# facebookresearch/brainmagick

Measured on AMD Instinct MI355X. Metric: segments/s, 208-ch x 360-sample SimpleConv + ClipLoss training step, higher is better.
Workload: dtype f32 (fp32-accurate: operands split into 2 scaled f16 planes, 3 MFMA products, fp32 accumulate; same parity tolerances as exact fp32, see DESIGN.md §2); 1 GPU; cfg2: gwilliams2022-shaped MEG C=208 T=360, F=120 features, 27 subjects, clip_conv SimpleConv (8985590 params) + ClipLoss + Adam; batch_per_gpu=256, global_batch=256, negatives=local, parallelism=dp1, comm=none, rccl_world=1, candidate_gather=none, distinct_batches=8

## Files before the change

brainmagick_amd/csrc/clip.hip:

```cpp
#include "bm_common.h"

__global__ __launch_bounds__(256) void inv_norms_kernel(const float* __restrict__ cand, long K,
                                                        float* __restrict__ inv_norm) {
    __shared__ double sh[4];
    const float* row = cand + (long)blockIdx.x * K;
    double s = 0;
    if ((K & 3) == 0) {
        float a0 = 0.f, a1 = 0.f, a2 = 0.f, a3 = 0.f;
        for (long i = threadIdx.x; i < K / 4; i += blockDim.x) {
            const float4 v = reinterpret_cast<const float4*>(row)[i];
            a0 += v.x * v.x; a1 += v.y * v.y; a2 += v.z * v.z; a3 += v.w * v.w;
        }
        s = (double)a0 + (double)a1 + (double)a2 + (double)a3;
    } else {
        float a = 0.f;
        for (long i = threadIdx.x; i < K; i += blockDim.x) a += row[i] * row[i];
        s = a;
    }
    s = bm_wave_sum_d(s);
    if ((threadIdx.x & 63) == 0) sh[threadIdx.x >> 6] = s;
    __syncthreads();
    if (threadIdx.x == 0) {
        const double t = sh[0] + sh[1] + sh[2] + sh[3];
        inv_norm[blockIdx.x] = 1.0f / (1e-8f + (float)sqrt(t));
// ... 359 lines not shown
}

extern "C" int bm_row_softmax(const float* x, float* y, int rows, int cols, void* stream) {
    BM_REQUIRE(x && y, "row_softmax: null pointer");
    if (rows == 0) return BM_OK;
    hipLaunchKernelGGL(row_softmax_kernel, dim3((rows + 3) / 4), dim3(256), 0, (hipStream_t)stream, x, y, rows, cols);
    return bm_check_launch("row_softmax");
}

__global__ __launch_bounds__(256) void rowwise_dot_kernel(const float* __restrict__ a, const float* __restrict__ b,
                                                          const float* __restrict__ scale, float* __restrict__ out,
                                                          long K) {
    __shared__ double sh[4];
    const float* ar = a + (long)blockIdx.x * K;
    const float* br = b + (long)blockIdx.x * K;
    float s = 0.f;
    for (long i = threadIdx.x; i < K; i += blockDim.x) s += ar[i] * br[i];
    double d = bm_wave_sum_d((double)s);
    if ((threadIdx.x & 63) == 0) sh[threadIdx.x >> 6] = d;
    __syncthreads();
    if (threadIdx.x == 0) out[blockIdx.x] = (float)(sh[0] + sh[1] + sh[2] + sh[3]) * (scale ? scale[blockIdx.x] : 1.f);
}

extern "C" int bm_rowwise_dot(const float* a, const float* b, const float* scale, float* out, int rows, long K,
                              void* stream) {
    BM_REQUIRE(a && b && out, "rowwise_dot: null pointer");
    if (rows == 0) return BM_OK;
    hipLaunchKernelGGL(rowwise_dot_kernel, dim3(rows), dim3(256), 0, (hipStream_t)stream, a, b, scale, out, K);
    return bm_check_launch("rowwise_dot");
}

__global__ void segment_sum_cols_kernel(const float* __restrict__ p, const int* __restrict__ order,
                                        const int* __restrict__ seg, float* __restrict__ pv, int rows,
                                        int cols, int V) {
    const int lane = threadIdx.x & 63;
    const int row = blockIdx.x * (blockDim.x >> 6) + (threadIdx.x >> 6);
    if (row >= rows) return;
    const float* pr = p + (long)row * cols;
    for (int v = lane; v < V; v += 64) {
        float s = 0.f;
        for (int k = seg[v]; k < seg[v + 1]; ++k) s += pr[order[k]];
        pv[(long)row * V + v] = s;
    }
}

extern "C" int bm_segment_sum_cols(const float* p, const int* order, const int* seg, float* pv, int rows,
                                   int cols, int V, void* stream) {
    BM_REQUIRE(p && order && seg && pv, "segment_sum_cols: null pointer");
    if (rows == 0 || V == 0) return BM_OK;
    hipLaunchKernelGGL(segment_sum_cols_kernel, dim3((rows + 3) / 4), dim3(256), 0, (hipStream_t)stream, p, order,
                       seg, pv, rows, cols, V);
    return bm_check_launch("segment_sum_cols");
}
```

brainmagick_amd/csrc/pack.hip:

```cpp
#include "bm_common.h"

__global__ void pack_weights_kernel(const float* __restrict__ src, float* __restrict__ dst, int G,
                                    int M, int Cin, int KS, long sg, long sm, long sc, long sj,
                                    int flip, int Mpad, int nchunk, const float* alpha_ptr) {
    const long total = (long)G * nchunk * KS * BM_BKC * Mpad;
    const float alpha = alpha_ptr ? *alpha_ptr : 1.f;
    for (long i = (long)blockIdx.x * blockDim.x + threadIdx.x; i < total;
         i += (long)gridDim.x * blockDim.x) {
        long r = i;
        const int m = (int)(r % Mpad); r /= Mpad;
        const int cc = (int)(r % BM_BKC); r /= BM_BKC;
        const int j = (int)(r % KS); r /= KS;
        const int chunk = (int)(r % nchunk);
        const int g = (int)(r / nchunk);
        const int c = chunk * BM_BKC + cc;
        float v = 0.f;
        if (m < M && c < Cin) {
            const int jj = flip ? KS - 1 - j : j;
            v = alpha * src[g * sg + m * sm + c * sc + jj * sj];
        }
        dst[i] = v;
    }
}

// ... 60 lines not shown

extern "C" int bm_group_by_index(const long* idx, int B, int G, int* order, int* seg, int* err_flag,
                                 void* stream) {
    BM_REQUIRE(seg && ((idx && order) || B == 0), "group_by_index: null pointer");
    BM_REQUIRE(B >= 0 && G > 0, "group_by_index: bad dims B=%d G=%d", B, G);
    BM_REQUIRE((long)G + 1 + B <= BM_GROUP_MAX_INTS, "group_by_index: B + G + 1 = %ld ints of LDS exceed the %d of a "
               "launch (B=%d G=%d)", (long)G + 1 + B, BM_GROUP_MAX_INTS, B, G);
    hipLaunchKernelGGL(group_by_index_kernel, dim3(1), dim3(256), (size_t)(G + 1 + B) * sizeof(int),
                       (hipStream_t)stream, idx, B, G, order, seg, err_flag);
    return bm_check_launch("group_by_index");
}

__global__ void index_to_i32_kernel(const long* __restrict__ idx, int B, int G, int* __restrict__ out,
                                    int* __restrict__ err) {
    const int i = blockIdx.x * blockDim.x + threadIdx.x;
    if (i >= B) return;
    long v = idx[i];
    if (v < 0 || v >= G) {
        if (err) atomicExch(err, 1);
        v = 0;
    }
    out[i] = (int)v;
}

extern "C" int bm_index_to_i32(const long* idx, int B, int G, int* out, int* err_flag, void* stream) {
    BM_REQUIRE((idx && out) || B == 0, "index_to_i32: null pointer");
    BM_REQUIRE(B >= 0 && G > 0, "index_to_i32: bad dims B=%d G=%d", B, G);
    if (B == 0) return BM_OK;
    hipLaunchKernelGGL(index_to_i32_kernel, dim3((B + 255) / 256), dim3(256), 0, (hipStream_t)stream, idx, B,
                       G, out, err_flag);
    return bm_check_launch("index_to_i32");
}

__global__ void reduce_splits_kernel(const float* __restrict__ part, float* __restrict__ out, int G,
                                     int nsplit, int M, int Cn, int KS, long sg, long sm, long sc,
                                     long sj) {
    const long N = (long)Cn * KS;
    const long per = (long)M * N;
    const long total = (long)G * per;
    for (long i = (long)blockIdx.x * blockDim.x + threadIdx.x; i < total;
         i += (long)gridDim.x * blockDim.x) {
        const int g = (int)(i / per);
        const long r = i - (long)g * per;
        const int m = (int)(r / N);
        const int n = (int)(r - (long)m * N);
        const int c = n / KS, j = n - c * KS;
        const float* p = part + (long)g * nsplit * per + r;
        float s = 0.f;
        for (int k = 0; k < nsplit; ++k) s += p[(long)k * per];
        out[g * sg + m * sm + c * sc + j * sj] = s;
    }
}

__global__ void reduce_splits_vec4_kernel(const float* __restrict__ part, float* __restrict__ out, int G,
                                          int nsplit, int M, int Cn, int KS, long sg, long sm, long sc,
                                          long sj) {
    const long N = (long)Cn * KS;
    const long per = (long)M * N;
    const long total4 = (long)G * per / 4;
    for (long i4 = (long)blockIdx.x * blockDim.x + threadIdx.x; i4 < total4;
         i4 += (long)gridDim.x * blockDim.x) {
        const long i = i4 * 4;
        const int g = (int)(i / per);
        const long r = i - (long)g * per;
        const float* p = part + (long)g * nsplit * per + r;
        float4 s = make_float4(0.f, 0.f, 0.f, 0.f);
// ... 62 lines not shown
```

brainmagick_amd/functional.py:

```python

import torch

from . import hip_ops as H



ACT_CODES = {"none": H.ACT_NONE, "gelu": H.ACT_GELU, "relu": H.ACT_RELU, "leaky": H.ACT_LEAKY}


def _c(t: torch.Tensor) -> torch.Tensor:
    return t if t.is_contiguous() else t.contiguous()


_arange_cache = {}


def _arange_i32(n: int, device, repeat: int = 1) -> torch.Tensor:
    key = (n, repeat, device.type, device.index)
    t = _arange_cache.get(key)
    if t is None:
        if len(_arange_cache) > 64:
            _arange_cache.clear()
        t = torch.arange(n, dtype=torch.int32, device=device)
        if repeat != 1:
# ... 219 lines not shown
        U, C, O, D = ctx.dims
        dout = _c(dout)
        B, _, T = meg.shape
        dheads = None
        if ctx.needs_input_grad[1]:
            order, seg = H.group_by_index(_c(layout_index.to(torch.int64)), U)
            dweights = H.gemm_nt(dout, meg, B, O, C, T, 1, 1, order=order, seg=seg, G=U).view(U, O, C)
            dscores = H.softmax_bwd(weights, dweights)
            wp = H.pack_weights(dscores, U, O, C, 1, O * C, C, 1, 0, shape=(D, 1))
            uidx = _arange_i32(U, meg.device)
            _, per_layout, _ = H.conv_nn(emb, wp, O, 1, 1, widx=uidx)
            if ctx.per_layout_heads:
                dheads = per_layout
            else:
                dheads = H.sum_over_batch(per_layout) if U > 1 else per_layout[0]
        dmeg = None
        if ctx.needs_input_grad[0]:
            wpt = H.pack_weights(weights, U, C, O, 1, O * C, 1, C, 0, shape=(T, 1))
            _, dmeg, _ = H.conv_nn(dout, wpt, C, 1, 1, widx=widx)
        return dmeg, dheads, None, None, None, None


class FusedFrontEndFn(torch.autograd.Function):

    @staticmethod
    def forward(ctx, meg, heads, w1, b1, ws, positions_u, layout_index, subjects, ban_center, ban_radius: float):
        meg, heads, w1, ws, positions_u = _c(meg), _c(heads), _c(w1), _c(ws), _c(positions_u)
        U, C, _ = positions_u.shape
        O, Dp = heads.shape
        L = w1.shape[0]
        S, _, D = ws.shape
        B, _, T = meg.shape
        dev = meg.device
        emb = H.fourier_emb(positions_u, Dp)
        seg_u = _arange_i32(U + 1, dev)
        scores = H.gemm_nt(heads, emb, U, O, C, Dp, a_strides=(0, Dp), x_strides=(C * Dp, Dp), seg=seg_u,
                           G=U).view(U, O, C)
        wm = H.masked_softmax(scores, positions_u, ban_center, ban_radius)
        _, p, _ = H.conv_nn(wm, H.pack_conv_fwd(w1), L, 1, 1)
        bcol = (b1 if b1 is not None else torch.zeros(L, device=dev)).view(1, L, 1).expand(U, L, 1)
        xp = torch.cat([p, bcol], dim=2).repeat_interleave(S, dim=0).contiguous()
        widx_p = _arange_i32(S, dev, repeat=U)
        _, wc, _ = H.conv_nn(xp, H.pack_weights(ws, S, D, L, 1, L * D, 1, D, 0), D, 1, 1, widx=widx_p)
        bias_c = wc[:, :, C].contiguous()
        pair = H.index_i32(_c(layout_index.to(torch.int64)), U) * S + H.index_i32(_c(subjects.to(torch.int64)), S)
        wpc = H.pack_weights(wc, U * S, D, C, 1, D * (C + 1), C + 1, 1, 0, shape=(T, 1))
        _, out, _ = H.conv_nn(meg, wpc, D, 1, 1, widx=pair, bias=bias_c, bias_gstride=D)
        ctx.save_for_backward(meg, emb, wm, xp, ws, w1, pair, widx_p, wc)
        ctx.dims = (U, C, O, Dp, L, S, D)
        ctx.has_b1 = b1 is not None
        return out

    @staticmethod
    def backward(ctx, dout):
        meg, emb, wm, xp, ws, w1, pair, widx_p, wc = ctx.saved_tensors
        U, C, O, Dp, L, S, D = ctx.dims
        dout = _c(dout)
        B, _, T = meg.shape
        dev = meg.device
        P = U * S
        order, seg = H.group_by_index(pair.to(torch.int64), P)
        gaug = torch.empty(P, D, C + 1, device=dev, dtype=torch.float32)
        H.gemm_nt(dout, meg, B, D, C, T, 1, 1, order=order, seg=seg, G=P, out=gaug,
                  out_strides=(D * (C + 1), C + 1, 1, 0))
        gaug[:, :, C] = H.segment_sum_cols(H.time_sums_t(dout), order, seg).t()
        seg_p = _arange_i32(P + 1, dev)
        dws = dw1 = db1 = dheads = None
        if ctx.needs_input_grad[4]:
            t1 = H.gemm_nt(xp, gaug, P, L, D, C + 1, seg=seg_p, G=P)
            dws = (H.sum_over_batch(t1.view(U, S * L * D)) if U > 1 else t1).view(S, L, D)
        _, a, _ = H.conv_nn(gaug, H.pack_weights(ws, S, L, D, 1, L * D, D, 1, 0), L, 1, 1, widx=widx_p)
        a_u = torch.stack([H.sum_over_batch(a[u * S:(u + 1) * S]) for u in range(U)])
        if ctx.has_b1 and ctx.needs_input_grad[3]:
            db1 = H.sum_over_batch(a_u[:, :, C].contiguous()) if U > 1 else a_u[0, :, C].contiguous()
        if ctx.needs_input_grad[2]:
            dw1 = H.gemm_nt(a_u, wm, U, L, O, C, 1, 1, a_strides=(L * (C + 1), C + 1),
                            x_strides=(O * C, C)).view(L, O, 1)
        if ctx.needs_input_grad[1]:
            _, dwm, _ = H.conv_nn(a_u, H.pack_conv_dgrad(w1), O, 1, 1)
            dscores = H.softmax_bwd(wm, dwm[:, :, :C].contiguous())
            wp = H.pack_weights(dscores, U, O, C, 1, O * C, C, 1, 0, shape=(Dp, 1))
            uidx = _arange_i32(U, dev)
            _, per_layout, _ = H.conv_nn(emb, wp, O, 1, 1, widx=uidx)
            dheads = H.sum_over_batch(per_layout) if U > 1 else per_layout[0]
        dmeg = None
        if ctx.needs_input_grad[0]:
            wpt = H.pack_weights(wc, P, C, D, 1, D * (C + 1), 1, C + 1, 0, shape=(T, 1))
            _, dmeg, _ = H.conv_nn(dout, wpt, C, 1, 1, widx=pair)
        return dmeg, dheads, dw1, db1, dws, None, None, None, None, None


_CLIP_BLOCK_BYTES = 0x3f000000


def _candidate_blocks(Bc: int, K: int):
    if Bc * K * 4 < _CLIP_BLOCK_BYTES:
        return [(0, Bc)]
    rows = max(1, _CLIP_BLOCK_BYTES // (K * 4))
    if rows >= 128:
        rows -= rows % 128
    return [(r0, min(rows, Bc - r0)) for r0 in range(0, Bc, rows)]


def _clip_raw_scores(estimate, candidate, B, Bc, K):
    blocks = _candidate_blocks(Bc, K)
    if len(blocks) == 1:
        return H.gemm_nt_partials(estimate, candidate, 1, B, Bc, K, (0, K), (0, K))
    raw = torch.empty(1, B, Bc, device=estimate.device, dtype=torch.float32)
    cand2 = candidate.view(Bc, K)
    for r0, rows in blocks:
        blk = H.share_amax(candidate, cand2[r0:r0 + rows])
        H.gemm_nt(estimate, blk, 1, B, rows, K, 1, 1, a_strides=(0, K), x_strides=(0, K),
                  out=raw.view(-1)[r0:], out_strides=(0, Bc, 1, 0))
    return raw


class ClipLossFn(torch.autograd.Function):

    @staticmethod
    def forward(ctx, estimate, candidate, target_offset: int = 0, col_valid=None, symmetric: bool = False,
                normalize: bool = True):
        estimate, candidate = _c(estimate), _c(candidate)
# ... 199 lines not shown
```

brainmagick_amd/hip_ops.py:

```python
import ctypes
import typing as tp

import torch

from ._lib import lib, check, BmHipError

ACT_NONE, ACT_GELU, ACT_RELU, ACT_LEAKY = 0, 1, 2, 3
BKC = 16

import os as _os
DEFAULT_COMPUTE_DTYPE = "f16x2"
COMPUTE_DTYPES = ("f32", "f32x3", "f16x2")
_compute_dtype = _os.environ.get("BM_COMPUTE_DTYPE", DEFAULT_COMPUTE_DTYPE)
if _compute_dtype not in COMPUTE_DTYPES:
    raise ValueError(f"BM_COMPUTE_DTYPE must be one of {COMPUTE_DTYPES}, got {_compute_dtype!r}")


def set_compute_dtype(name: str):
    global _compute_dtype
    if name not in COMPUTE_DTYPES:
        raise ValueError(f"compute dtype must be one of {COMPUTE_DTYPES}, got {name!r}")
    _compute_dtype = name


# ... 36 lines not shown

def set_kernel_timer(timer: tp.Optional[KernelTimer]):
    global _timer
    _timer = timer


def _timed(label, flops: float, launch):
    if _timer is None:
        return launch()
    return _timer.launch(label() if callable(label) else label, flops, launch)


def _p(t: tp.Optional[torch.Tensor]):
    return None if t is None else ctypes.c_void_p(t.data_ptr())


def _stream():
    return ctypes.c_void_p(torch.cuda.current_stream().cuda_stream)


def _req(t: torch.Tensor, name: str, dtype=torch.float32):
    if not isinstance(t, torch.Tensor) or not t.is_cuda:
        raise BmHipError(f"{name}: expected a GPU tensor; the brainmagick_amd hot path has no CPU "
                         "fallback (got %s)" % (t.device if isinstance(t, torch.Tensor) else type(t)))
    if t.dtype != dtype:
        raise BmHipError(f"{name}: expected dtype {dtype}, got {t.dtype}")
    if not t.is_contiguous():
        raise BmHipError(f"{name}: expected a contiguous tensor")
    return t


def _opt(t, name, dtype=torch.float32):
    return None if t is None else _req(t, name, dtype)


def conv_mpad(M: int) -> int:
    return lib().bm_conv_mpad(M)


def _note(t: torch.Tensor, attr: str, value, *checked):
    try:
        setattr(t, attr, (t._version, t.data_ptr(), value) + checked)
        t._bm_epoch = _weights_epoch
    except Exception:
        pass


def _noted(t: torch.Tensor, attr: str, need_checked: bool = False):
    note = getattr(t, attr, None)
    if note is not None and note[0] == t._version and note[1] == t.data_ptr() and (not need_checked or note[3]) and \
            (not (t.requires_grad and t.is_leaf) or getattr(t, "_bm_epoch", None) == _weights_epoch):
        return note[2]
    return None


AMAX_SHARDS = 8
amax_scans = 0


def amax(x: torch.Tensor, nonfinite_flag: tp.Optional[torch.Tensor] = None) -> torch.Tensor:
    cached = _noted(x, "_bm_amax", nonfinite_flag is not None)
    if cached is not None:
        return cached
    _req(x, "amax.x")
    global amax_scans
    amax_scans += 1
# ... 312 lines not shown


_index_err: tp.Dict[torch.device, torch.Tensor] = {}
_CHECK_INDICES_NOW = _os.environ.get("BM_CHECK_INDICES", "0") == "1"


def index_error_flag(device) -> torch.Tensor:
    device = torch.device(device)
    if device.index is None:
        device = torch.device("cuda", torch.cuda.current_device())
    flag = _index_err.get(device)
    if flag is None:
        flag = torch.zeros(3, device=device, dtype=torch.int32)
        _index_err[device] = flag
    return flag


def raise_if_index_error(device=None):
    flags = list(_index_err.values()) if device is None else [index_error_flag(device)]
    for flag in flags:
        if int(flag[0].item()) != 0:
            flag[0:1].zero_()
            raise IndexError("subject / layout index out of range for the weight table "
                             "(bm/models/common.py:57 would raise in `weights.gather`)")


def index_i32(idx: torch.Tensor, G: int) -> torch.Tensor:
    _req(idx, "index_i32.idx", torch.int64)
    out = torch.empty(idx.numel(), device=idx.device, dtype=torch.int32)
    check(lib().bm_index_to_i32(_p(idx), idx.numel(), G, _p(out), _p(index_error_flag(idx.device)),
                                _stream()), "bm_index_to_i32")
    if _CHECK_INDICES_NOW:
        raise_if_index_error(idx.device)
    return out


def group_by_index(idx: torch.Tensor, G: int):
    _req(idx, "group_by_index.idx", torch.int64)
    B = idx.numel()
    order = torch.empty(B, device=idx.device, dtype=torch.int32)
    seg = torch.empty(G + 1, device=idx.device, dtype=torch.int32)
    check(lib().bm_group_by_index(_p(idx), B, G, _p(order), _p(seg), _p(index_error_flag(idx.device)),
                                  _stream()), "bm_group_by_index")
    return order, seg


_NT_SUFFIX = {"f32": "", "f32x3": "_x3"}


def _nt_plan(M, Cn, KS, S, T, G, dil, grouped, a_strides, x_strides, nsplit=None, partials=False):
    L = lib()
    family, swapped = _compute_dtype, False
    if family == "f16x2":
        family = "f32x3"
        if partials:
            if L.bm_gemm_nt_h2_covers(M, Cn, 1, S, T, 1, 1, 0):
                dense = S == 1 and tuple(a_strides) == (0, T) and tuple(x_strides) == (0, T)
                family = "scores" if dense and L.bm_clip_scores_h2_covers(M, Cn, T) else "h2"
        elif a_strides[1] == T and x_strides[1] == T and \
                (S == 1 or (a_strides[0] == M * T and x_strides[0] == Cn * T)):
            covered = bool(L.bm_gemm_nt_h2_covers(M, Cn, KS, S, T, G, dil, int(grouped)))
            swapped = not covered and KS == 1 and bool(L.bm_gemm_nt_h2_covers(Cn, M, KS, S, T, G, dil, int(grouped)))
            if swapped:
                M, Cn = Cn, M
            if covered or swapped:
                family = "h2_grouped" if grouped else "h2_rows"
# ... 87 lines not shown


_direct_armed = _DirectArmed()


class direct_grads_armed:

    def __enter__(self):
        _direct_armed.depth += 1
        return self

    def __exit__(self, *exc):
        _direct_armed.depth -= 1
        return False


def grad_destination(param: torch.Tensor) -> tp.Optional[torch.Tensor]:
    dst = getattr(param, "_bm_grad_dst", None)
    if dst is None or dst[1][0] or param.grad is not None or not _direct_armed.on:
        return None
    dst[1][0] = True
    return dst[0]


def gemm_nt_partials(a, x, S, M, Cn, T, a_strides, x_strides, nsplit=None):
    _req(a, "gemm_nt.a")
    _req(x, "gemm_nt.x")
    family, _, nsplit = _nt_plan(M, Cn, 1, S, T, 1, 1, False, a_strides, x_strides, nsplit, partials=True)
    part = torch.empty(nsplit, M, Cn, device=a.device, dtype=torch.float32)
    _nt_launch(family, "clip_scores:gemm_nt{}", a, x, part, S, 1, M, Cn, T, 1, 1, a_strides, x_strides, None, None, nsplit)
    return part


def sum_over_batch(x: torch.Tensor) -> torch.Tensor:
    _req(x, "sum_over_batch.x")
    B = x.shape[0]
    out = torch.empty(x.shape[1:], device=x.device, dtype=torch.float32)
    check(lib().bm_sum_over_batch(_p(x), _p(out), B, out.numel(), _stream()), "bm_sum_over_batch")
    return out


def bn_finalize(stats, count: int, gamma, beta, running_mean, running_var, num_batches,
                momentum: float, eps: float):
    _req(stats, "bn_finalize.stats")
    channel_major = getattr(stats, "_bm_channel_major", False)
    (C, ntiles, _) = stats.shape if channel_major else (stats.shape[1], stats.shape[0], 2)
    mean, invstd, scale, shift = (torch.empty(C, device=stats.device, dtype=torch.float32)
                                  for _ in range(4))
    check((lib().bm_bn_finalize_cm if channel_major else lib().bm_bn_finalize)(_p(stats), ntiles, C, count, _p(_opt(gamma, "gamma")),
                               _p(_opt(beta, "beta")), _p(_opt(running_mean, "running_mean")),
                               _p(_opt(running_var, "running_var")),
                               _p(_opt(num_batches, "num_batches", torch.int64)), momentum, eps,
                               _p(mean), _p(invstd), _p(scale), _p(shift), _stream()),
          "bm_bn_finalize")
    return mean, invstd, scale, shift


def bn_eval_affine(gamma, beta, running_mean, running_var, eps: float):
    _req(running_mean, "running_mean")
    C = running_mean.numel()
    mean, invstd, scale, shift = (torch.empty(C, device=running_mean.device, dtype=torch.float32)
                                  for _ in range(4))
    check(lib().bm_bn_eval_affine(C, _p(_opt(gamma, "gamma")), _p(_opt(beta, "beta")),
                                  _p(running_mean), _p(_req(running_var, "running_var")), eps,
                                  _p(mean), _p(invstd), _p(scale), _p(shift), _stream()),
          "bm_bn_eval_affine")
# ... 422 lines not shown
    if cardinality > MAX_CATEGORY_CARDINALITY:
        raise ValueError(f"category_counts: cardinality {cardinality} exceeds the cap of {MAX_CATEGORY_CARDINALITY} "
                         "bins (the histogram lives in LDS)")
    _req(x, "category_counts.x")
    if x.dim() != 3:
        raise BmHipError(f"category_counts: x {tuple(x.shape)} must be [N, F, T]")
    mask, mode = _regress_mask(mask, x.shape, "category_counts")
    N, F, T = x.shape
    counts = torch.zeros(cardinality, device=x.device, dtype=torch.float32)
    flags = torch.zeros(1, device=x.device, dtype=torch.int32)
    ws = torch.zeros(lib().bm_category_counts_workspace_bytes(cardinality), device=x.device, dtype=torch.uint8)
    check(lib().bm_category_counts(_p(x), _p(mask), mode, N, F, T, f, cardinality, _p(counts), _p(flags), _p(ws),
                                   ws.numel(), _stream()), "bm_category_counts")
    return counts, flags


def row_softmax(x: torch.Tensor) -> torch.Tensor:
    _req(x, "row_softmax.x")
    y = torch.empty_like(x)
    check(lib().bm_row_softmax(_p(x), _p(y), x.shape[0], x.shape[1], _stream()), "bm_row_softmax")
    return y


def rowwise_dot(a: torch.Tensor, b: torch.Tensor, scale=None) -> torch.Tensor:
    _req(a, "rowwise_dot.a")
    _req(b, "rowwise_dot.b")
    rows = a.shape[0]
    out = torch.empty(rows, device=a.device, dtype=torch.float32)
    check(lib().bm_rowwise_dot(_p(a), _p(b), _p(_opt(scale, "scale")), _p(out), rows,
                               a.numel() // max(rows, 1), _stream()), "bm_rowwise_dot")
    return out


def segment_sum_cols(p: torch.Tensor, order: torch.Tensor, seg: torch.Tensor) -> torch.Tensor:
    _req(p, "segment_sum_cols.p")
    rows, cols = p.shape
    V = seg.numel() - 1
    pv = torch.empty(rows, V, device=p.device, dtype=torch.float32)
    check(lib().bm_segment_sum_cols(_p(p), _p(_req(order, "order", torch.int32)),
                                    _p(_req(seg, "seg", torch.int32)), _p(pv), rows, cols, V, _stream()),
          "bm_segment_sum_cols")
    return pv


def topk_rows(x: torch.Tensor, k: int, col_labels=None, row_labels=None):
    _req(x, "topk_rows.x")
    N, V = x.shape
    idx = torch.empty(N, k, device=x.device, dtype=torch.int32)
    val = torch.empty(N, k, device=x.device, dtype=torch.float32)
    hits = torch.empty(N, device=x.device, dtype=torch.int32) if col_labels is not None else None
    check(lib().bm_topk_rows(_p(x), N, V, k, _p(idx), _p(val),
                             _p(_opt(col_labels, "col_labels", torch.int64)),
                             _p(_opt(row_labels, "row_labels", torch.int64)), _p(hits), _stream()),
          "bm_topk_rows")
    return idx, val, hits


def adam_step(param, grad, exp_avg, exp_avg_sq, step: int, lr: float, beta1: float, beta2: float,
              eps: float, grad_scale: float = 1.0):
    for t, n in ((param, "param"), (grad, "grad"), (exp_avg, "exp_avg"), (exp_avg_sq, "exp_avg_sq")):
        _req(t, f"adam_step.{n}")
    check(lib().bm_adam_step(_p(param), _p(grad), _p(exp_avg), _p(exp_avg_sq), param.numel(), step,
                             lr, beta1, beta2, eps, grad_scale, _stream()), "bm_adam_step")
    for t in (param, exp_avg, exp_avg_sq):
        _touched(t)
    weights_changed()


def _per_dir(ts, name=None, shape=None):
    if name is not None:
        for t in ts:
            _req(t, name)
            assert tuple(t.shape) == shape, (name, tuple(t.shape), shape)
    return [_p(t) for t in ts] + [None] * (2 - len(ts))

# ... 41 lines not shown
```

include/bm_hip.h:

```cpp
#ifndef BM_HIP_H
#define BM_HIP_H
#ifdef __cplusplus
extern "C" {
#endif

#define BM_ACT_NONE 0
#define BM_ACT_GELU 1
#define BM_ACT_RELU 2
#define BM_ACT_LEAKY 3

int bm_version(void);
const char* bm_last_error(void);
int bm_device_count(void);

int bm_conv_mt_for(int M);
int bm_conv_mpad(int M);
int bm_conv_stats_tiles(int B, int T);
long bm_packed_weight_elems(int G, int M, int Cin, int KS);
int bm_pack_weights(const float* src, float* dst, int G, int M, int Cin, int KS, long sg, long sm,
                    long sc, long sj, int flip, const float* alpha_ptr, void* stream);
int bm_group_by_index(const long* idx, int B, int G, int* order, int* seg, int* err_flag, void* stream);
int bm_index_to_i32(const long* idx, int B, int G, int* out, int* err_flag, void* stream);
int bm_reduce_splits(const float* part, float* out, int G, int nsplit, int M, int Cn, int KS, long sg,
                     long sm, long sc, long sj, void* stream);
int bm_sum_over_batch(const float* x, float* out, int B, long n, void* stream);

int bm_conv1d_nn(const float* x, long x_bstride, const float* wpacked, const int* widx,
                 const float* bias, long bias_gstride, const float* ep_scale, const float* ep_shift, const float* res,
                 long res_bstride, float* y_pre, float* y_out, long y_bstride, float* stats, int B,
                 int Cin, int M, int T, int KS, int dil, int act, float leak, void* stream);

int bm_conv1d_out_len(int T, int KS, int stride, int dil, int pad, int transposed);
int bm_conv_strided_stats_tiles(int B, int Tout, int stride, int transposed);
int bm_conv1d_strided(const float* x, long x_bstride, const float* wpacked, const float* bias,
                      const float* ep_scale, const float* ep_shift, float* y_pre, float* y_out, long y_bstride,
                      float* stats, int B, int Cin, int M, int T, int Tout, int KS, int stride, int dil, int pad,
                      int act, float leak, void* stream);
int bm_conv1d_transposed(const float* x, long x_bstride, const float* wpacked, const float* bias,
                         const float* ep_scale, const float* ep_shift, float* y_pre, float* y_out, long y_bstride,
                         float* stats, int B, int Cin, int M, int T, int Tout, int KS, int stride, int dil, int pad,
                         int act, float leak, void* stream);
int bm_conv1d_strided_wgrad_suggest_splits(int R, int Q, int KS, int S, int U);
int bm_conv1d_strided_wgrad(const float* a, long a_sstride, const float* xl, long xl_sstride, float* part, int S,
                            int R, int Q, int U, int L, int KS, int stride, int dil, int pad, int nsplit,
                            void* stream);

int bm_lstm_layer_fwd(const float* whh0, const float* whh1, const float* gx0, const float* gx1, float* y,
                      float* gates0, float* gates1, float* c0, float* c1, int H, int B, int T, int dirs,
                      void* stream);
int bm_lstm_layer_bwd(const float* whh0, const float* whh1, const float* dy, const float* gates0,
                      const float* gates1, const float* c0, const float* c1, float* dg0, float* dg1,
                      float* dc0, float* dc1, int H, int B, int T, int dirs, void* stream);

long bm_packed_weight_elems_x3(int G, int M, int Cin, int KS);
int bm_pack_weights_x3(const float* src, void* dst, int G, int M, int Cin, int KS, long sg, long sm,
// ... 128 lines not shown

long bm_regress_workspace_bytes(void);
int bm_regress_loss_fwd(const float* est, const float* out, const unsigned char* mask, int mask_mode, int B, int F,
                        int T, int kind, float* loss, double* count, void* workspace, long workspace_bytes, int* flag,
                        void* stream);
int bm_regress_loss_bwd(const float* est, const float* out, const unsigned char* mask, int mask_mode, int B, int F,
                        int T, int kind, const float* grad_out, const double* count, float* d_est, float* d_out,
                        float* amax_out, float* amax_rows_out, void* workspace, long workspace_bytes, void* stream);
int bm_regress_metric_update(const float* est, long est_bstride, const float* out, long out_bstride,
                             const unsigned char* mask, long mask_bstride, int mask_full, int B, int F, int T, int t0,
                             double* acc, void* stream);

int bm_feature_decoding_fwd(const float* est, const float* out, const unsigned char* mask, const float* weights,
                            long n_weights, const int* table, int n_features, int B, int C, int Co, int T, float* loss,
                            float* terms, double* denoms, float* lse, void* workspace, long workspace_bytes, int* flag,
                            void* stream);
int bm_feature_decoding_bwd(const float* est, const float* out, const unsigned char* mask, const float* weights,
                            long n_weights, const int* table, int n_features, int B, int C, int Co, int T,
                            const float* grad_out, const double* denoms, const float* lse, float* d_est, void* stream);
int bm_class_acc_update(const float* est, long est_bstride, const float* target, long target_bstride,
                        const unsigned char* mask, long mask_bstride, int B, int K, int T, int t0, long* acc,
                        void* stream);

int bm_clip_cand_coef(const float* dscaled, const float* scores, const float* inv_norm,
                      const float* alpha, float* coef, int B, int Bc, void* stream);
int bm_row_axpy_sub(float* y, const float* x, const float* coef, int rows, long K, void* stream);
int bm_topk_rows(const float* x, int rows, int cols, int k, int* idx_out, float* val_out,
                 const long* col_labels, const long* row_labels, int* hit_out, void* stream);

int bm_row_softmax(const float* x, float* y, int rows, int cols, void* stream);
int bm_rowwise_dot(const float* a, const float* b, const float* scale, float* out, int rows, long K,
                   void* stream);
int bm_segment_sum_cols(const float* p, const int* order, const int* seg, float* pv, int rows, int cols,
                        int V, void* stream);

int bm_adam_step(float* param, const float* grad, float* exp_avg, float* exp_avg_sq, long n, int step,
                 double lr, double beta1, double beta2, double eps, double grad_scale, void* stream);

int bm_comm_unique_id_bytes(void);
int bm_comm_available(void);
int bm_comm_unique_id(void* out_id);
int bm_comm_init(const void* id, int world, int rank, int device, void** handle);
int bm_comm_destroy(void* handle);
int bm_comm_world(void* handle);
int bm_comm_rank(void* handle);
int bm_comm_reported_world(void* handle);
int bm_comm_reported_rank(void* handle);
int bm_comm_allgather(void* handle, const float* send, float* recv, long count, void* stream);
int bm_comm_reduce_scatter(void* handle, const float* send, float* recv, long count, void* stream);
int bm_comm_allreduce(void* handle, const float* send, float* recv, long count, int op, void* stream);

#ifdef __cplusplus
}
#endif
#endif
```

Before: 16440 segments/s.

## Compose front-end weights with a dedicated strided small-GEMM MFMA kernel

```diff
diff --git a/brainmagick_amd/csrc/clip.hip b/brainmagick_amd/csrc/clip.hip
--- a/brainmagick_amd/csrc/clip.hip
+++ b/brainmagick_amd/csrc/clip.hip
@@ -415,7 +415,7 @@
 
 __global__ void segment_sum_cols_kernel(const float* __restrict__ p, const int* __restrict__ order,
                                         const int* __restrict__ seg, float* __restrict__ pv, int rows,
-                                        int cols, int V) {
+                                        int cols, int V, long s_row, long s_col) {
     const int lane = threadIdx.x & 63;
     const int row = blockIdx.x * (blockDim.x >> 6) + (threadIdx.x >> 6);
     if (row >= rows) return;
@@ -423,15 +423,16 @@
     for (int v = lane; v < V; v += 64) {
         float s = 0.f;
         for (int k = seg[v]; k < seg[v + 1]; ++k) s += pr[order[k]];
-        pv[(long)row * V + v] = s;
+        pv[row * s_row + v * s_col] = s;
     }
 }
 
 extern "C" int bm_segment_sum_cols(const float* p, const int* order, const int* seg, float* pv, int rows,
-                                   int cols, int V, void* stream) {
+                                   int cols, int V, long s_row, long s_col, void* stream) {
     BM_REQUIRE(p && order && seg && pv, "segment_sum_cols: null pointer");
+    BM_REQUIRE(s_row > 0 && s_col > 0, "segment_sum_cols: output strides must be positive (%ld, %ld)", s_row, s_col);
     if (rows == 0 || V == 0) return BM_OK;
     hipLaunchKernelGGL(segment_sum_cols_kernel, dim3((rows + 3) / 4), dim3(256), 0, (hipStream_t)stream, p, order,
-                       seg, pv, rows, cols, V);
+                       seg, pv, rows, cols, V, s_row, s_col);
     return bm_check_launch("segment_sum_cols");
 }
diff --git a/brainmagick_amd/csrc/pack.hip b/brainmagick_amd/csrc/pack.hip
--- a/brainmagick_amd/csrc/pack.hip
+++ b/brainmagick_amd/csrc/pack.hip
@@ -116,6 +116,32 @@
     return bm_check_launch("index_to_i32");
 }
 
+__global__ void pair_index_kernel(const long* __restrict__ layout, const long* __restrict__ subject, int B, int U,
+                                  int S, int* __restrict__ out, int* __restrict__ err) {
+    const int i = blockIdx.x * blockDim.x + threadIdx.x;
+    if (i >= B) return;
+    long u = layout[i], s = subject[i];
+    if (u < 0 || u >= U) {
+        if (err) atomicExch(err, 1);
+        u = 0;
+    }
+    if (s < 0 || s >= S) {
+        if (err) atomicExch(err, 1);
+        s = 0;
+    }
+    out[i] = (int)(u * S + s);
+}
+
+extern "C" int bm_pair_index(const long* layout, const long* subject, int B, int U, int S, int* out, int* err_flag,
+                             void* stream) {
+    BM_REQUIRE((layout && subject && out) || B == 0, "pair_index: null pointer");
+    BM_REQUIRE(B >= 0 && U > 0 && S > 0 && (long)U * S < (1L << 31), "pair_index: bad dims B=%d U=%d S=%d", B, U, S);
+    if (B == 0) return BM_OK;
+    hipLaunchKernelGGL(pair_index_kernel, dim3((B + 255) / 256), dim3(256), 0, (hipStream_t)stream, layout, subject,
+                       B, U, S, out, err_flag);
+    return bm_check_launch("pair_index");
+}
+
 __global__ void reduce_splits_kernel(const float* __restrict__ part, float* __restrict__ out, int G,
                                      int nsplit, int M, int Cn, int KS, long sg, long sm, long sc,
                                      long sj) {
diff --git a/brainmagick_amd/csrc/small_gemm.hip b/brainmagick_amd/csrc/small_gemm.hip
--- /dev/null
+++ b/brainmagick_amd/csrc/small_gemm.hip
@@ -0,0 +1,190 @@
+#include "bm_common.h"
+
+#define SG_KC 256
+#define SG_THREADS 512
+
+struct SmallGemmArgs {
+    const float* a; long sag, sar, sam, sak;
+    const float* b; long sbg, sbr, sbk, sbn;
+    float* c; long scg, scm, scn;
+    const float* bias;
+    float* c2; long s2g, s2m; int col2;
+    int R, M, N, K, RK;
+    int a_kfast, b_kfast;
+    int rinc, kinc;
+};
+
+struct SgWalk {
+    int kk, k;
+    long off, wrap, chunk;
+};
+
+__device__ __forceinline__ SgWalk sg_walk(bool kfast, long sr, long sk, const SmallGemmArgs& p, int tid) {
+    SgWalk w;
+    w.kk = kfast ? (tid & 255) : (tid >> 5) * 16;
+    const int r = w.kk / p.K;
+    w.k = w.kk - r * p.K;
+    w.off = r * sr + w.k * sk;
+    w.wrap = sr - p.K * sk;
+    w.chunk = p.rinc * sr + p.kinc * sk;
+    return w;
+}
+
+__device__ __forceinline__ void sg_load(float (&v)[16], const float* base, bool kfast, SgWalk& w, long sx, long sk,
+                                        int x0, int nx, const SmallGemmArgs& p, int tid) {
+    if (kfast) {
+        const float* pk = base + w.off;
+        const bool kin = w.kk < p.RK;
+#pragma unroll
+        for (int i = 0; i < 16; ++i) {
+            const int x = x0 + (tid >> 8) + 2 * i;
+            v[i] = (kin && x < nx) ? pk[x * sx] : 0.f;
+        }
+    } else {
+        const int x = x0 + (tid & 31);
+        const float* px = base + x * sx;
+        const bool xin = x < nx;
+        int k = w.k;
+        long o = w.off;
+#pragma unroll
+        for (int i = 0; i < 16; ++i) {
+            v[i] = (xin && w.kk + i < p.RK) ? px[o] : 0.f;
+            ++k;
+            o += sk;
+            if (k == p.K) {
+                k = 0;
+                o += w.wrap;
+            }
+        }
+    }
+    w.kk += SG_KC;
+    w.k += p.kinc;
+    w.off += w.chunk;
+    if (w.k >= p.K) {
+        w.k -= p.K;
+        w.off += w.wrap;
+    }
+}
+
+__device__ __forceinline__ int sg_lds(int slot, int x) { return slot * 32 + (x ^ (slot & 31)); }
+
+__device__ __forceinline__ void sg_stage(float* s, const float (&v)[16], bool kfast, int tid) {
+    if (kfast) {
+#pragma unroll
+        for (int i = 0; i < 16; ++i) s[sg_lds(tid & 255, (tid >> 8) + 2 * i)] = v[i];
+    } else {
+#pragma unroll
+        for (int i = 0; i < 16; ++i) s[sg_lds((tid >> 5) * 16 + i, tid & 31)] = v[i];
+    }
+}
+
+__global__ __launch_bounds__(SG_THREADS) void small_gemm_kernel(SmallGemmArgs p) {
+    __shared__ float smem[2 * SG_KC * 32];
+    float* As = smem;
+    float* Bs = smem + SG_KC * 32;
+
+    const int tid = threadIdx.x;
+    const int lane = tid & 63;
+    const int wave = tid >> 6;
+    const int nl = lane & 31;
+    const int h = lane >> 5;
+    const int n0 = blockIdx.x * 32;
+    const int m0 = blockIdx.y * 32;
+    const int g = blockIdx.z;
+    const float* ag = p.a + g * p.sag;
+    const float* bg = p.b + g * p.sbg;
+    const bool akf = p.a_kfast != 0, bkf = p.b_kfast != 0;
+
+    f32x16 acc;
+#pragma unroll
+    for (int r = 0; r < 16; ++r) acc[r] = 0.f;
+
+    SgWalk wa = sg_walk(akf, p.sar, p.sak, p, tid);
+    SgWalk wb = sg_walk(bkf, p.sbr, p.sbk, p, tid);
+    float a0[16], b0[16], a1[16], b1[16];
+    const int nchunk = (p.RK + SG_KC - 1) / SG_KC;
+#define SG_LOAD(A_, B_)                                              \
+    {                                                                \
+        sg_load(A_, ag, akf, wa, p.sam, p.sak, m0, p.M, p, tid);     \
+        sg_load(B_, bg, bkf, wb, p.sbn, p.sbk, n0, p.N, p, tid);     \
+    }
+#define SG_STEP(A_, B_, MORE_)                                                                               \
+    {                                                                                                        \
+        sg_stage(As, A_, akf, tid);                                                                          \
+        sg_stage(Bs, B_, bkf, tid);                                                                          \
+        __syncthreads();                                                                                     \
+        if (MORE_) SG_LOAD(A_, B_)                           \
+        _Pragma("unroll") for (int kk = 0; kk < 16; ++kk) {                                                  \
+            const int slot = wave * 32 + 2 * kk + h;                                                         \
+            acc = __builtin_amdgcn_mfma_f32_32x32x2f32(As[sg_lds(slot, nl)], Bs[sg_lds(slot, nl)], acc, 0, 0, 0); \
+        }                                                                                                    \
+        __syncthreads();                                                                                     \
+    }
+    SG_LOAD(a0, b0)
+    if (nchunk > 1) SG_LOAD(a1, b1)
+    for (int c = 0; c < nchunk; c += 2) {
+        SG_STEP(a0, b0, c + 2 < nchunk)
+        if (c + 1 < nchunk) SG_STEP(a1, b1, c + 3 < nchunk)
+    }
+#undef SG_STEP
+#undef SG_LOAD
+
+    float* red = smem;
+#pragma unroll
+    for (int r = 0; r < 16; ++r) red[(wave * 16 + r) * 64 + lane] = acc[r];
+    __syncthreads();
+    const int n = n0 + nl;
+    float* cg = p.c + g * p.scg;
+    float* c2g = p.c2 ? p.c2 + g * p.s2g : nullptr;
+#pragma unroll
+    for (int q = 0; q < 2; ++q) {
+        const int r = 2 * wave + q;
+        const int m = m0 + (r & 3) + 8 * (r >> 2) + 4 * h;
+        if (m < p.M && n < p.N) {
+            float s = red[r * 64 + lane];
+#pragma unroll
+            for (int w = 1; w < 8; ++w) s += red[(w * 16 + r) * 64 + lane];
+            cg[m * p.scm + n * p.scn] = s;
+            if (c2g && n == p.col2) c2g[m * p.s2m] = s;
+        }
+    }
+    if (p.bias && blockIdx.x == 0 && tid < 32) {
+        const int m = m0 + tid;
+        if (m < p.M) {
+            const float v = p.bias[m];
+            cg[m * p.scm + p.N * p.scn] = v;
+            if (c2g && p.col2 == p.N) c2g[m * p.s2m] = v;
+        }
+    }
+}
+
+extern "C" int bm_small_gemm(const float* a, long sag, long sar, long sam, long sak, const float* b, long sbg, long sbr,
+                             long sbk, long sbn, float* c, long scg, long scm, long scn, const float* bias, float* c2,
+                             long s2g, long s2m, int col2, int G, int R, int M, int N, int K, void* stream) {
+    BM_REQUIRE(a && b && c, "small_gemm: null pointer");
+    BM_REQUIRE(G > 0 && R > 0 && M > 0 && N > 0 && K > 0, "small_gemm: bad dims G=%d R=%d M=%d N=%d K=%d", G, R, M, N, K);
+    BM_REQUIRE(sag >= 0 && sar >= 0 && sam >= 0 && sak >= 0 && sbg >= 0 && sbr >= 0 && sbk >= 0 && sbn >= 0,
+               "small_gemm: negative operand stride");
+    BM_REQUIRE(scg >= 0 && scm > 0 && scn > 0, "small_gemm: output strides must be positive (scg=%ld scm=%ld scn=%ld)",
+               scg, scm, scn);
+    BM_REQUIRE((long)R * K < (1L << 31) - SG_KC, "small_gemm: reduction of %ld terms is too long", (long)R * K);
+    BM_REQUIRE(cdiv(M, 32) <= 65535 && G <= 65535, "small_gemm: M=%d or G=%d exceeds the grid", M, G);
+    if (c2) {
+        BM_REQUIRE(s2g >= 0 && s2m > 0, "small_gemm: second-output strides must be positive (s2g=%ld s2m=%ld)", s2g, s2m);
+        BM_REQUIRE(col2 >= 0 && col2 < N + (bias ? 1 : 0), "small_gemm: col2=%d outside the %d columns", col2,
+                   N + (bias ? 1 : 0));
+    }
+    SmallGemmArgs p;
+    p.a = a; p.sag = sag; p.sar = sar; p.sam = sam; p.sak = sak;
+    p.b = b; p.sbg = sbg; p.sbr = sbr; p.sbk = sbk; p.sbn = sbn;
+    p.c = c; p.scg = scg; p.scm = scm; p.scn = scn;
+    p.bias = bias; p.c2 = c2; p.s2g = s2g; p.s2m = s2m; p.col2 = col2;
+    p.R = R; p.M = M; p.N = N; p.K = K; p.RK = R * K;
+    p.a_kfast = sak == 1 && sam != 1;
+    p.b_kfast = sbk == 1 && sbn != 1;
+    p.rinc = SG_KC / K;
+    p.kinc = SG_KC % K;
+    const dim3 grid((unsigned)cdiv(N, 32), (unsigned)cdiv(M, 32), (unsigned)G);
+    hipLaunchKernelGGL(small_gemm_kernel, grid, dim3(SG_THREADS), 0, (hipStream_t)stream, p);
+    return bm_check_launch("small_gemm");
+}
diff --git a/brainmagick_amd/functional.py b/brainmagick_amd/functional.py
--- a/brainmagick_amd/functional.py
+++ b/brainmagick_amd/functional.py
@@ -275,7 +275,40 @@
         S, _, D = ws.shape
         B, _, T = meg.shape
         dev = meg.device
+        ctx.gemm_chain = H.front_end_gemm()
         emb = H.fourier_emb(positions_u, Dp)
+        if ctx.gemm_chain:
+            scores = torch.empty(U, O, C, device=dev, dtype=torch.float32)
+            H.small_gemm(heads.view(1, 1, O, Dp).expand(U, 1, O, Dp), emb.view(U, 1, C, Dp).transpose(2, 3), scores)
+            wm = H.masked_softmax(scores, positions_u, ban_center, ban_radius)
+            xp = torch.empty(U, L, C + 1, device=dev, dtype=torch.float32)
+            H.small_gemm(w1.view(1, 1, L, O).expand(U, 1, L, O), wm.view(U, 1, O, C), xp[:, :, :C],
+                         bias=b1 if b1 is not None else torch.zeros(L, device=dev))
+            wc = torch.empty(U * S, D, C + 1, device=dev, dtype=torch.float32)
+            bias_c = torch.empty(U * S, D, device=dev, dtype=torch.float32)
+            for u in range(U):
+                H.small_gemm(ws.transpose(1, 2).unsqueeze(1), xp[u].view(1, 1, L, C + 1).expand(S, 1, L, C + 1),
+                             wc[u * S:(u + 1) * S], col_out=bias_c[u * S:(u + 1) * S], col=C)
+            pair = H.pair_index(_c(layout_index.to(torch.int64)), _c(subjects.to(torch.int64)), U, S)
+            widx_p = pair
+        else:
+            scores, wm, xp, wc, bias_c, pair, widx_p = FusedFrontEndFn._compose_x3(
+                heads, emb, w1, b1, ws, positions_u, layout_index, subjects, ban_center, ban_radius)
+        wpc = H.pack_weights(wc, U * S, D, C, 1, D * (C + 1), C + 1, 1, 0, shape=(T, 1))
+        _, out, _ = H.conv_nn(meg, wpc, D, 1, 1, widx=pair, bias=bias_c, bias_gstride=D)
+        ctx.save_for_backward(meg, emb, wm, xp, ws, w1, pair, widx_p, wc)
+        ctx.dims = (U, C, O, Dp, L, S, D)
+        ctx.has_b1 = b1 is not None
+        ctx.params = (heads, w1, ws)
+        return out
+
+    @staticmethod
+    def _compose_x3(heads, emb, w1, b1, ws, positions_u, layout_index, subjects, ban_center, ban_radius):
+        U, C, _ = positions_u.shape
+        O, Dp = heads.shape
+        L = w1.shape[0]
+        S, _, D = ws.shape
+        dev = heads.device
         seg_u = _arange_i32(U + 1, dev)
         scores = H.gemm_nt(heads, emb, U, O, C, Dp, a_strides=(0, Dp), x_strides=(C * Dp, Dp), seg=seg_u,
                            G=U).view(U, O, C)
@@ -287,12 +320,15 @@
         _, wc, _ = H.conv_nn(xp, H.pack_weights(ws, S, D, L, 1, L * D, 1, D, 0), D, 1, 1, widx=widx_p)
         bias_c = wc[:, :, C].contiguous()
         pair = H.index_i32(_c(layout_index.to(torch.int64)), U) * S + H.index_i32(_c(subjects.to(torch.int64)), S)
-        wpc = H.pack_weights(wc, U * S, D, C, 1, D * (C + 1), C + 1, 1, 0, shape=(T, 1))
-        _, out, _ = H.conv_nn(meg, wpc, D, 1, 1, widx=pair, bias=bias_c, bias_gstride=D)
-        ctx.save_for_backward(meg, emb, wm, xp, ws, w1, pair, widx_p, wc)
-        ctx.dims = (U, C, O, Dp, L, S, D)
-        ctx.has_b1 = b1 is not None
-        return out
+        return scores, wm, xp, wc, bias_c, pair, widx_p
+
+    @staticmethod
+    def _grad_out(param, shape, dev):
+        dst = H.grad_destination(param)
+        if dst is None:
+            out = torch.empty(shape, device=dev, dtype=torch.float32)
+            return out, out
+        return dst, dst.view(shape)
 
     @staticmethod
     def backward(ctx, dout):
@@ -306,7 +342,49 @@
         gaug = torch.empty(P, D, C + 1, device=dev, dtype=torch.float32)
         H.gemm_nt(dout, meg, B, D, C, T, 1, 1, order=order, seg=seg, G=P, out=gaug,
                   out_strides=(D * (C + 1), C + 1, 1, 0))
-        gaug[:, :, C] = H.segment_sum_cols(H.time_sums_t(dout), order, seg).t()
+        if ctx.gemm_chain:
+            H.segment_sum_cols(H.time_sums_t(dout), order, seg, out=gaug[:, :, C].t())
+            dws, dw1, db1, dheads = FusedFrontEndFn._chain_backward_gemm(ctx, gaug, emb, wm, xp, ws, w1)
+        else:
+            gaug[:, :, C] = H.segment_sum_cols(H.time_sums_t(dout), order, seg).t()
+            dws, dw1, db1, dheads = FusedFrontEndFn._chain_backward_x3(ctx, gaug, emb, wm, xp, ws, w1, widx_p)
+        dmeg = None
+        if ctx.needs_input_grad[0]:
+            wpt = H.pack_weights(wc, P, C, D, 1, D * (C + 1), 1, C + 1, 0, shape=(T, 1))
+            _, dmeg, _ = H.conv_nn(dout, wpt, C, 1, 1, widx=pair)
+        return dmeg, dheads, dw1, db1, dws, None, None, None, None, None
+
+    @staticmethod
+    def _chain_backward_gemm(ctx, gaug, emb, wm, pb, ws, w1):
+        U, C, O, Dp, L, S, D = ctx.dims
+        dev = gaug.device
+        g4 = gaug.view(U, S, D, C + 1)
+        dws = dw1 = db1 = dheads = None
+        if ctx.needs_input_grad[4]:
+            out, dws = FusedFrontEndFn._grad_out(ctx.params[2], (S, L, D), dev)
+            H.small_gemm(pb.view(1, U, L, C + 1).expand(S, U, L, C + 1), g4.permute(1, 0, 3, 2), out.view(S, L, D))
+        a_u = torch.empty(U, L, C + 1, device=dev, dtype=torch.float32)
+        want_db1 = ctx.has_b1 and ctx.needs_input_grad[3]
+        db1_u = torch.empty(U, L, device=dev, dtype=torch.float32) if want_db1 else None
+        H.small_gemm(ws.view(1, S, L, D).expand(U, S, L, D), g4, a_u, col_out=db1_u, col=C)
+        if want_db1:
+            db1 = H.sum_over_batch(db1_u) if U > 1 else db1_u[0]
+        if ctx.needs_input_grad[2]:
+            out, dw1 = FusedFrontEndFn._grad_out(ctx.params[1], (L, O, 1), dev)
+            H.small_gemm(a_u[:, :, :C].unsqueeze(0), wm.transpose(1, 2).unsqueeze(0), out.view(1, L, O))
+        if ctx.needs_input_grad[1]:
+            dwm = torch.empty(U, O, C, device=dev, dtype=torch.float32)
+            H.small_gemm(w1.view(1, 1, L, O).transpose(2, 3).expand(U, 1, O, L), a_u[:, :, :C].unsqueeze(1), dwm)
+            dscores = H.softmax_bwd(wm, dwm)
+            out, dheads = FusedFrontEndFn._grad_out(ctx.params[0], (O, Dp), dev)
+            H.small_gemm(dscores.unsqueeze(0), emb.unsqueeze(0), out.view(1, O, Dp))
+        return dws, dw1, db1, dheads
+
+    @staticmethod
+    def _chain_backward_x3(ctx, gaug, emb, wm, xp, ws, w1, widx_p):
+        U, C, O, Dp, L, S, D = ctx.dims
+        dev = gaug.device
+        P = U * S
         seg_p = _arange_i32(P + 1, dev)
         dws = dw1 = db1 = dheads = None
         if ctx.needs_input_grad[4]:
@@ -326,11 +404,7 @@
             uidx = _arange_i32(U, dev)
             _, per_layout, _ = H.conv_nn(emb, wp, O, 1, 1, widx=uidx)
             dheads = H.sum_over_batch(per_layout) if U > 1 else per_layout[0]
-        dmeg = None
-        if ctx.needs_input_grad[0]:
-            wpt = H.pack_weights(wc, P, C, D, 1, D * (C + 1), 1, C + 1, 0, shape=(T, 1))
-            _, dmeg, _ = H.conv_nn(dout, wpt, C, 1, 1, widx=pair)
-        return dmeg, dheads, dw1, db1, dws, None, None, None, None, None
+        return dws, dw1, db1, dheads
 
 
 _CLIP_BLOCK_BYTES = 0x3f000000
diff --git a/brainmagick_amd/hip_ops.py b/brainmagick_amd/hip_ops.py
--- a/brainmagick_amd/hip_ops.py
+++ b/brainmagick_amd/hip_ops.py
@@ -92,6 +92,16 @@
 
 def _opt(t, name, dtype=torch.float32):
     return None if t is None else _req(t, name, dtype)
+
+
+def _strided(t: torch.Tensor, name: str, shape=None):
+    if not isinstance(t, torch.Tensor) or not t.is_cuda:
+        raise BmHipError(f"{name}: expected a GPU tensor; the brainmagick_amd hot path has no CPU fallback")
+    if t.dtype != torch.float32:
+        raise BmHipError(f"{name}: expected dtype torch.float32, got {t.dtype}")
+    if shape is not None and tuple(t.shape) != tuple(shape):
+        raise BmHipError(f"{name}: expected shape {tuple(shape)}, got {tuple(t.shape)}")
+    return t
 
 
 def conv_mpad(M: int) -> int:
@@ -470,6 +480,19 @@
                                 _stream()), "bm_index_to_i32")
     if _CHECK_INDICES_NOW:
         raise_if_index_error(idx.device)
+    return out
+
+
+def pair_index(layout: torch.Tensor, subject: torch.Tensor, U: int, S: int) -> torch.Tensor:
+    _req(layout, "pair_index.layout", torch.int64)
+    _req(subject, "pair_index.subject", torch.int64)
+    if layout.numel() != subject.numel():
+        raise BmHipError(f"pair_index: {layout.numel()} layout indices for {subject.numel()} subjects")
+    out = torch.empty(layout.numel(), device=layout.device, dtype=torch.int32)
+    check(lib().bm_pair_index(_p(layout), _p(subject), layout.numel(), U, S, _p(out),
+                              _p(index_error_flag(layout.device)), _stream()), "bm_pair_index")
+    if _CHECK_INDICES_NOW:
+        raise_if_index_error(layout.device)
     return out
 
 
@@ -623,6 +646,44 @@
     return part
 
 
+_front_end_gemm = _os.environ.get("BM_FRONT_END_GEMM", "1") != "0"
+
+
+def set_front_end_gemm(on: bool) -> bool:
+    global _front_end_gemm
+    old, _front_end_gemm = _front_end_gemm, bool(on)
+    return old
+
+
+def front_end_gemm() -> bool:
+    return _front_end_gemm
+
+
+def small_gemm(a: torch.Tensor, b: torch.Tensor, out: torch.Tensor, bias: tp.Optional[torch.Tensor] = None,
+               col_out: tp.Optional[torch.Tensor] = None, col: int = 0) -> torch.Tensor:
+    _strided(a, "small_gemm.a")
+    _strided(b, "small_gemm.b")
+    if a.dim() != 4 or b.dim() != 4 or a.shape[:2] != b.shape[:2] or a.shape[3] != b.shape[2]:
+        raise BmHipError(f"small_gemm: a {tuple(a.shape)} and b {tuple(b.shape)} are not [G, R, M, K] and [G, R, K, N]")
+    G, R, M, K = a.shape
+    N = b.shape[3]
+    _strided(out, "small_gemm.out", (G, M, N))
+    _touched(out)
+    if bias is not None and bias.numel() != M:
+        raise BmHipError(f"small_gemm: bias of {bias.numel()} elements for {M} rows")
+    c2 = (0, 0)
+    if col_out is not None:
+        _strided(col_out, "small_gemm.col_out", (G, M))
+        c2 = col_out.stride()
+
+    def launch():
+        check(lib().bm_small_gemm(_p(a), *a.stride(), _p(b), *b.stride(), _p(out), *out.stride(), _p(_opt(bias, "bias")),
+                                  _p(col_out), *c2, col, G, R, M, N, K, _stream()), "bm_small_gemm")
+    nt = b.stride(2) == 1 and b.stride(3) != 1
+    _timed("gemm_nt_sg_kernel" if nt else "conv_nn_sg_kernel", 2.0 * G * R * M * N * K, launch)
+    return out
+
+
 def sum_over_batch(x: torch.Tensor) -> torch.Tensor:
     _req(x, "sum_over_batch.x")
     B = x.shape[0]
@@ -1111,15 +1172,20 @@
     return out
 
 
-def segment_sum_cols(p: torch.Tensor, order: torch.Tensor, seg: torch.Tensor) -> torch.Tensor:
+def segment_sum_cols(p: torch.Tensor, order: torch.Tensor, seg: torch.Tensor,
+                     out: tp.Optional[torch.Tensor] = None) -> torch.Tensor:
     _req(p, "segment_sum_cols.p")
     rows, cols = p.shape
     V = seg.numel() - 1
-    pv = torch.empty(rows, V, device=p.device, dtype=torch.float32)
+    if out is None:
+        out = torch.empty(rows, V, device=p.device, dtype=torch.float32)
+    else:
+        _strided(out, "segment_sum_cols.out", (rows, V))
+        _touched(out)
     check(lib().bm_segment_sum_cols(_p(p), _p(_req(order, "order", torch.int32)),
-                                    _p(_req(seg, "seg", torch.int32)), _p(pv), rows, cols, V, _stream()),
-          "bm_segment_sum_cols")
-    return pv
+                                    _p(_req(seg, "seg", torch.int32)), _p(out), rows, cols, V, out.stride(0),
+                                    out.stride(1), _stream()), "bm_segment_sum_cols")
+    return out
 
 
 def topk_rows(x: torch.Tensor, k: int, col_labels=None, row_labels=None):
diff --git a/include/bm_hip.h b/include/bm_hip.h
--- a/include/bm_hip.h
+++ b/include/bm_hip.h
@@ -21,6 +21,8 @@
                     long sc, long sj, int flip, const float* alpha_ptr, void* stream);
 int bm_group_by_index(const long* idx, int B, int G, int* order, int* seg, int* err_flag, void* stream);
 int bm_index_to_i32(const long* idx, int B, int G, int* out, int* err_flag, void* stream);
+int bm_pair_index(const long* layout, const long* subject, int B, int U, int S, int* out, int* err_flag,
+                  void* stream);
 int bm_reduce_splits(const float* part, float* out, int G, int nsplit, int M, int Cn, int KS, long sg,
                      long sm, long sc, long sj, void* stream);
 int bm_sum_over_batch(const float* x, float* out, int B, long n, void* stream);
@@ -215,7 +217,11 @@
 int bm_rowwise_dot(const float* a, const float* b, const float* scale, float* out, int rows, long K,
                    void* stream);
 int bm_segment_sum_cols(const float* p, const int* order, const int* seg, float* pv, int rows, int cols,
-                        int V, void* stream);
+                        int V, long s_row, long s_col, void* stream);
+
+int bm_small_gemm(const float* a, long sag, long sar, long sam, long sak, const float* b, long sbg, long sbr,
+                  long sbk, long sbn, float* c, long scg, long scm, long scn, const float* bias, float* c2,
+                  long s2g, long s2m, int col2, int G, int R, int M, int N, int K, void* stream);
 
 int bm_adam_step(float* param, const float* grad, float* exp_avg, float* exp_avg_sq, long n, int step,
                  double lr, double beta1, double beta2, double eps, double grad_scale, void* stream);
```

Result: no change. 16510 segments/s, median of 2 (+0.4%).
